# NeLy-EPFL/flygym

Hardware: AMD Instinct MI355X
Metric: env-steps/sec (whole node), 4096 flies per GPU, flat terrain (higher is better)
Workload: dtype f32

## Files before the change

### flygym_amd/csrc/nmf_device.h

```cpp
#pragma once
#include <hip/hip_runtime.h>
#include <stdint.h>

#include <type_traits>
#include <utility>

#include "nmf_families.h"

namespace nmf {

constexpr int kMaxCon = 48;
constexpr int kActHistWords = 64;
constexpr float kMinVal = 1e-15f;

enum { GEOM_CAPSULE = 0, GEOM_HULL = 1 };
enum { ACT_POSITION = 0, ACT_ADHESION = 1, ACT_MOTOR = 2 };

__device__ __forceinline__ int opaque(int v) { asm volatile("" : "+v"(v)); return v; }

template <int... I, class F>
__device__ __forceinline__ void static_for_impl(std::integer_sequence<int, I...>, F&& f) {
  (f(std::integral_constant<int, I>{}), ...);
}
template <int N, class F>
// ... 228 lines not shown
  *cs = ((q + 1) & 2) ? -cc : cc;
}

__device__ __forceinline__ void sym6_add_inertia(Sym6& A, const float* I) {
  A.v[sym_idx(0, 0)] += I[4]; A.v[sym_idx(1, 1)] += I[5]; A.v[sym_idx(2, 2)] += I[6];
  A.v[sym_idx(0, 1)] += I[7]; A.v[sym_idx(0, 2)] += I[8]; A.v[sym_idx(1, 2)] += I[9];
  float hx = I[1], hy = I[2], hz = I[3];
  A.v[sym_idx(0, 4)] += -hz; A.v[sym_idx(0, 5)] += hy;
  A.v[sym_idx(1, 3)] += hz;  A.v[sym_idx(1, 5)] += -hx;
  A.v[sym_idx(2, 3)] += -hy; A.v[sym_idx(2, 4)] += hx;
  A.v[sym_idx(3, 3)] += I[0]; A.v[sym_idx(4, 4)] += I[0]; A.v[sym_idx(5, 5)] += I[0];
}

#define NMF_DPP(v, ctrl) __builtin_bit_cast(float, __builtin_amdgcn_update_dpp(0, __builtin_bit_cast(int, (v)), (ctrl), 0xf, 0xf, true))
#define NMF_PIN(v) asm("" : "+v"(v))
__device__ __forceinline__ float grp8_sum(float v) {
  NMF_PIN(v);
  v += NMF_DPP(v, 0xB1);
  v += NMF_DPP(v, 0x4E);
  v += NMF_DPP(v, 0x141);
  NMF_PIN(v);
  return v;
}

#define NMF_DPP_ROWS(v, ctrl, rows) __builtin_bit_cast(float, __builtin_amdgcn_update_dpp(0, __builtin_bit_cast(int, (v)), (ctrl), (rows), 0xf, false))
__device__ __forceinline__ float wave_sum(float v) {
  v += NMF_DPP(v, 0xB1);
  v += NMF_DPP(v, 0x4E);
  v += NMF_DPP(v, 0x141);
  v += NMF_DPP(v, 0x140);
  v += NMF_DPP_ROWS(v, 0x142, 0xa);
  v += NMF_DPP_ROWS(v, 0x143, 0xc);
  return __builtin_bit_cast(float, __builtin_amdgcn_readlane(__builtin_bit_cast(int, v), 63));
}
template <int I>
__device__ __forceinline__ float grp8_bcast(float v) {
  constexpr int pattern = 0x18 | (I << 5);
  return __builtin_bit_cast(float, __builtin_amdgcn_ds_swizzle(__builtin_bit_cast(int, v), pattern));
}
typedef float f32x4 __attribute__((ext_vector_type(4)));
__device__ __forceinline__ float grp8_lo(float v) {
  return __builtin_bit_cast(float, __builtin_amdgcn_update_dpp(__builtin_bit_cast(int, v), __builtin_bit_cast(int, v), 0x114, 0xf, 0xa, false));
}
__device__ __forceinline__ float grp8_hi(float v) {
  return __builtin_bit_cast(float, __builtin_amdgcn_update_dpp(__builtin_bit_cast(int, v), __builtin_bit_cast(int, v), 0x104, 0xf, 0x5, false));
}
// ... 22 lines not shown
__device__ __forceinline__ int wave_reduce_bits(int v, int idn, Op op) {
  v = op(v, NMF_DPP_OLD(idn, v, 0xB1, 0xf));
  v = op(v, NMF_DPP_OLD(idn, v, 0x4E, 0xf));
  v = op(v, NMF_DPP_OLD(idn, v, 0x141, 0xf));
  v = op(v, NMF_DPP_OLD(idn, v, 0x140, 0xf));
  v = op(v, NMF_DPP_OLD(idn, v, 0x142, 0xa));
  v = op(v, NMF_DPP_OLD(idn, v, 0x143, 0xc));
  return __builtin_amdgcn_readlane(v, 63);
}
__device__ __forceinline__ float wave_min(float v) {
  return __builtin_bit_cast(float, wave_reduce_bits(__builtin_bit_cast(int, v), 0x7f800000, [](int a, int b) {
    return __builtin_bit_cast(int, fminf(__builtin_bit_cast(float, a), __builtin_bit_cast(float, b))); }));
}
__device__ __forceinline__ float wave_max(float v) {
  return __builtin_bit_cast(float, wave_reduce_bits(__builtin_bit_cast(int, v), (int)0xff800000, [](int a, int b) {
    return __builtin_bit_cast(int, fmaxf(__builtin_bit_cast(float, a), __builtin_bit_cast(float, b))); }));
}
__device__ __forceinline__ float groups_sum(float v) {
  v += NMF_DPP(v, 0x128);
  { float a = v, b = v; asm volatile("s_nop 1\n\tv_permlane16_swap_b32 %0, %1\n\ts_nop 1" : "+v"(a), "+v"(b)); v = a + b; }
  { float a = v, b = v; asm volatile("s_nop 1\n\tv_permlane32_swap_b32 %0, %1\n\ts_nop 1" : "+v"(a), "+v"(b)); v = a + b; }
  return v;
}
__device__ __forceinline__ int wave_prefix_min_int(int v) {
  constexpr int big = 0x7fffffff;
  auto mn = [](int a, int b) { return a < b ? a : b; };
  v = mn(v, NMF_DPP_OLD(big, v, 0x111, 0xf));
  v = mn(v, NMF_DPP_OLD(big, v, 0x112, 0xf));
  v = mn(v, NMF_DPP_OLD(big, v, 0x114, 0xf));
  v = mn(v, NMF_DPP_OLD(big, v, 0x118, 0xf));
  v = mn(v, NMF_DPP_OLD(big, v, 0x142, 0xa));
  v = mn(v, NMF_DPP_OLD(big, v, 0x143, 0xc));
  return v;
}
__device__ __forceinline__ int wave_min_int(int v) {
  return wave_reduce_bits(v, 0x7fffffff, [](int a, int b) { return a < b ? a : b; });
}
__device__ __forceinline__ void wave_argmin(float& v, int& i) {
  const float m = wave_min(v);
  i = wave_min_int(v == m ? i : 0x7fffffff);
  v = m;
}
__device__ __forceinline__ void wave_argmax(float& v, int& i) {
  const float m = wave_max(v);
  i = wave_min_int(v == m ? i : 0x7fffffff);
  v = m;
// ... 4 lines not shown
```

### flygym_amd/csrc/nmf_step.hip

```cpp
#include "nmf_device.h"
#include "nmf_step_lds.h"
#include "nmf_step_diag.h"
#include "nmf_tree_fwd.h"
#include "nmf_step_kinematics.h"
#include "nmf_step_collision.h"
#include "nmf_step_aba.h"
#include "nmf_step_contact.h"
#include "nmf_dual.h"
#include "nmf_step_noslip.h"
#include "nmf_step_actuation.h"
#include "nmf_step_forward.h"
#include "nmf_step_io.h"
#include "nmf_tree.h"

namespace nmf {

template <class TP> constexpr int waves_per_simd() { return 2; }

template <class TP>
__device__ __forceinline__ void stage_launch_constants(FlyLds<TP>& s, const GModel& m) {
  if constexpr (!TP::kStar) { if (threadIdx.x == 0) { s.rt_nb = m.nb; s.rt_nv = m.nv; } __syncthreads(); }
  if constexpr (TP::kNFact > 1) {
    for (int b = threadIdx.x; b < TP::kTblB && b < m.nb; b += kWave) {
      s.t_body[b] = (unsigned char)m.tree_body[b < m.tree_lvl_start[m.tree_nlevel] ? b : 0];
      s.t_parent[b] = (unsigned char)(b ? m.body_parent[b] : 0);
      s.t_dofadr[b] = (unsigned char)m.body_dofadr[b]; s.t_dofnum[b] = (unsigned char)m.body_dofnum[b];
      s.t_cstart[b] = (unsigned char)m.tree_child_start[b]; s.t_ccount[b] = (unsigned char)m.tree_child_count[b];
    }
    for (int j = threadIdx.x; j < TP::kTblV && j < m.nv; j += kWave) s.t_dofbody[j] = (unsigned char)m.dof_body[j];
    if (threadIdx.x < 18) s.t_lvl[threadIdx.x] = (unsigned char)m.tree_lvl_start[threadIdx.x];
    if (threadIdx.x == 0) s.t_nlevel = (unsigned char)m.tree_nlevel;
    if constexpr (TP::kStar) {
      for (int i = threadIdx.x; i < kRestLevels * 16; i += kWave) (&s.t_pack[0][0][0])[i] = m.rest_fast ? m.rest_pack[i] : 0xffffffffu;
    }
    __syncthreads();
  }
  const int lane = threadIdx.x;
  for (int j = lane; j < s.nv(); j += kWave) {
    if constexpr (row_width_s<TP>() > 6) s.S[j][6] = 0.f;
    s.arm[j] = m.dof_armature[j];
    if constexpr (kHasCm3<TP>) { s.damp[j] = m.dof_damping[j]; s.dlt[j] = m.dof_armature[j] + m.timestep * m.dof_damping[j]; }
  }
  if (lane < 6) {
    const KLane K = k_lane(lane, make_frame(v3(m.plane[0], m.plane[1], m.plane[2])));
    float* q = s.k_tab[lane];
#pragma unroll
    for (int i = 0; i < 3; ++i) { q[i] = K.dA[i]; q[3 + i] = K.dB[i]; q[6 + i] = K.dO[i]; }
    q[9] = __int_as_float(K.ia); q[10] = __int_as_float(K.ib);
    int words[3];
    inertia_map_pack(lane, words);
    q[11] = __int_as_float(words[0]); q[12] = __int_as_float(words[1]); q[13] = __int_as_float(words[2]);
    if constexpr (kHasIsym<TP>) {
#pragma unroll
      for (int c = 0; c < 6; c++) {
        const int i = lane < c ? lane : c, jx = lane < c ? c : lane;
        q[14 + c] = __int_as_float(sym_idx(i, jx));
      }
    }
  }
  if constexpr (kHasIsym<TP>) if (lane == 0) {
    const Frame fr = make_frame(v3(m.plane[0], m.plane[1], m.plane[2]));
    st3(&s.frame9[0], fr.n); st3(&s.frame9[3], fr.t1); st3(&s.frame9[6], fr.t2);
    HotModel& h = s.hot;
    h.dof_axis = m.dof_axis; h.body_pos = m.body_pos; h.body_quat = m.body_quat; h.geom_p0 = m.geom_p0; h.geom_p1 = m.geom_p1;
// ... 194 lines not shown
```

### flygym_amd/csrc/nmf_step_aba.h

```cpp
#pragma once
#include "nmf_device.h"

namespace nmf {

template <class TP>
__device__ __forceinline__ bool rest_reduced(const FlyLds<TP>& s) {
  if constexpr (TP::kStar) { if constexpr (TP::REST_B > 0) return __builtin_amdgcn_readfirstlane(s.reduced) != 0; }
  return false;
}
template <class TP, class F>
__device__ __forceinline__ void for_dofs(const FlyLds<TP>& s, bool red, int lane, F&& f) {
  if constexpr (TP::kStar) { if constexpr (TP::REST_V > 0) {
    if (red) { for (int jj = lane; jj < TP::NV - TP::REST_V; jj += kWave) f(jj < 6 ? jj : jj + TP::REST_V); return; }
  } }
  for (int j = lane; j < s.nv(); j += kWave) f(j);
}
template <class TP, class F>
__device__ __forceinline__ void for_bodies(const FlyLds<TP>& s, bool red, int lane, F&& f) {
  if constexpr (TP::kStar) { if constexpr (TP::REST_B > 0) {
    if (red) { for (int bb = lane; bb < TP::NB - TP::REST_B; bb += kWave) f(bb < 1 ? 0 : bb + TP::REST_B); return; }
  } }
  for (int b = lane; b < s.nb(); b += kWave) f(b);
}

// ... 45 lines not shown
    float pw[TP::NBL];
#pragma unroll
    for (int l = 0; l < TP::NBL; ++l) pw[l] = W[b0 + l][L.rr];
    static_for<TP::NBL>([&](auto I) {
      constexpr int l = TP::NBL - 1 - decltype(I)::value;
      acc += pw[l];
      W[b0 + l][L.rr] = acc;
    });
  }
  WSYNC();
  if (lane < 6) {
    float a0 = W[0][lane];
#pragma unroll
    for (int k = 0; k < TP::NLEG; ++k) a0 += W[TP::LB0 + k * TP::NBL][lane];
    if constexpr (TP::REST_B > 0) {
      if (!red) for (int k = (int)s.t_cstart[0]; k < (int)s.t_cstart[0] + (int)s.t_ccount[0]; ++k) a0 += W[(int)s.t_body[k]][lane];
    }
    W[0][lane] = a0;
  }
  WSYNC();
  if constexpr (TP::REST_V == 0 && TP::NV > kWave && TP::NV <= 2 * kWave) {
    const int jb = lane + kWave;
    const bool two = jb < TP::NV;
    const float pa = dot(ldsv(s.S[lane]), ldsv(W[dof_body_of<TP>(lane)]));
    float pb = 0.f;
    if (two) pb = dot(ldsv(s.S[jb]), ldsv(W[dof_body_of<TP>(jb)]));
    emit(lane, pa);
    if (two) emit(jb, pb);
  } else {
    for_dofs(s, red, lane, [&](int j) {
      emit(j, dot(ldsv(s.S[j]), ldsv(W[j >= TP::LD0 || j < 6 ? dof_body_of<TP>(j) : tbl_dofbody(s, j)])));
    });
  }
  WSYNC();
  }
}

template <class TP, class Emit>
__device__ __forceinline__ void mul_M(FlyLds<TP>& s, const float* x, const GModel& m, int lane, bool have_twists, Emit&& emit) {
  if (!have_twists) sweep_twists(s, x, s.T, m, lane);
  const bool red = rest_reduced(s);
  for_bodies(s, red, lane, [&](int b) {
    const SV tb = ldsv(s.T[b]);
    SV wb = inert_mul(s.Ib[b], tb);
    if constexpr (TP::kStar) { if constexpr (TP::REST_B > 0) { if (red && b == 0) wb = wb + rest_inertia_mul(s, tb); } }
    stsv(s.W[b], wb);
  });
  WSYNC();
  sweep_project(s, s.W, m, lane, [&](int j, float v) { emit(j, v + s.arm[j] * x[j]); });
}

constexpr int kInertiaIdx[6][6] = {{4, 7, 8, 0, 3, 2}, {7, 5, 9, 3, 0, 1}, {8, 9, 6, 2, 1, 0},
                                   {0, 3, 2, 0, 0, 0}, {3, 0, 1, 0, 0, 0}, {2, 1, 0, 0, 0, 0}};
constexpr int kInertiaSgn[6][6] = {{1, 1, 1, 0, -1, 1}, {1, 1, 1, 1, 0, -1}, {1, 1, 1, -1, 1, 0},
// ... 63 lines not shown
  if constexpr (kHasCm3<TP>) {
    const float* q = s.c_m3[c];
    m_nn = q[0]; m_n1 = q[1]; m_n2 = q[2]; m_11 = q[3]; m_22 = q[4];
    if (m_nn == 0.f) return;
  } else {
    const int act = info_act(s.c_info[c]);
    if (!act) return;
    const float D = s.c_D[c], mu = s.c_mu[c];
    const float a0 = (act & 1) ? 1.f : 0.f, a1 = (act & 2) ? 1.f : 0.f, a2 = (act & 4) ? 1.f : 0.f, a3 = (act & 8) ? 1.f : 0.f;
    const float Dm = D * mu, Dmm = Dm * mu;
    m_nn = D * (a0 + a1 + a2 + a3); m_n1 = Dm * (a0 - a1); m_n2 = Dm * (a2 - a3); m_11 = Dmm * (a0 + a1); m_22 = Dmm * (a2 + a3);
  }
  const V3 rc = ld3(s.c_r[c]);
  const float rcA = s.c_r[c][K.ia], rcB = s.c_r[c][K.ib];
  const float o_n = fmaf(rcA, K.dA[0], fmaf(-rcB, K.dB[0], K.dO[0]));
  const float o_1 = fmaf(rcA, K.dA[1], fmaf(-rcB, K.dB[1], K.dO[1]));
  const float o_2 = fmaf(rcA, K.dA[2], fmaf(-rcB, K.dB[2], K.dO[2]));
  const float C_n = m_nn * o_n + m_n1 * o_1 + m_n2 * o_2, C_1 = m_n1 * o_n + m_11 * o_1, C_2 = m_n2 * o_n + m_22 * o_2;
  const V3 w = C_n * fr.n + C_1 * fr.t1 + C_2 * fr.t2;
  const V3 x = cross(rc, w);
  row[0] += x.x; row[1] += x.y; row[2] += x.z; row[3] += w.x; row[4] += w.y; row[5] += w.z;
}

template <bool MFMA, bool MASKED>
__device__ __forceinline__ void aba_step_core(float (&IA)[6], float& pA, const float* sj, float sown, float mask, float delta, float tauj,
                                              float& U, float& u, float& invD, float& k) {
  f2 a01 = mk2(IA[0], IA[1]), a23 = mk2(IA[2], IA[3]), a45 = mk2(IA[4], IA[5]);
  f2 acc = a01 * mk2(sj[0], sj[1]);
  acc = __builtin_elementwise_fma(a23, mk2(sj[2], sj[3]), acc);
  acc = __builtin_elementwise_fma(a45, mk2(sj[4], sj[5]), acc);
  U = acc.x + acc.y;
  const float sr = MASKED ? mask * sown : sown;
  const float D = grp8_sum(sr * U) + delta;
  const float sp = grp8_sum(sr * pA);
  invD = __builtin_amdgcn_rcpf(D);
  u = tauj - sp;
  k = U * invD;
  if constexpr (MFMA) grp8_rank1_mfma(IA, -k, U);
  else {
    const f2 nk = mk2(-k, -k);
    a01 = __builtin_elementwise_fma(nk, mk2(grp8_bcast<0>(U), grp8_bcast<1>(U)), a01);
    a23 = __builtin_elementwise_fma(nk, mk2(grp8_bcast<2>(U), grp8_bcast<3>(U)), a23);
    a45 = __builtin_elementwise_fma(nk, mk2(grp8_bcast<4>(U), grp8_bcast<5>(U)), a45);
    IA[0] = a01.x; IA[1] = a01.y; IA[2] = a23.x; IA[3] = a23.y; IA[4] = a45.x; IA[5] = a45.y;
  }
  pA += k * u;
}
__device__ __forceinline__ void aba_step(float (&IA)[6], float& pA, const float* sj, float sown, float mask, float delta,
                                         float tauj, float& Uout, float& uout, float& invDout) {
  float U, k;
  aba_step_core<false, true>(IA, pA, sj, sown, mask, delta, tauj, U, uout, invDout, k);
  Uout = mask * U;
}
template <bool SHADOW0, bool MFMA = false>
__device__ __forceinline__ void aba_step_scaled(float (&IA)[6], float& pA, const float* sj, float sr, float mask, float delta,
                                                float tauj, float& UDout, float& uDout, float& Uraw, float& invDraw) {
  float u, k;
  aba_step_core<MFMA, false>(IA, pA, sj, sr, mask, delta, tauj, Uraw, u, invDraw, k);
  UDout = SHADOW0 ? k : mask * k; uDout = u * invDraw;
}
typedef const __attribute__((address_space(3))) float* lds_cptr;
template <class T>
__device__ __forceinline__ lds_cptr lds_pinned(const T* p) {
  lds_cptr q = (lds_cptr)(const void*)p;
  asm("" : "+v"(q));
  return q;
}

template <class TP> __device__ __forceinline__ float (*dual_leg(FlyLds<TP>& s))[8] {
// ... 210 lines not shown
  static_for<TP::NDL>([&](auto DD) {
    constexpr int d = TP::NDL - 1 - decltype(DD)::value;
    float sj[6], row[6];
#pragma unroll
    for (int i = 0; i < 6; i++) { sj[i] = n_sj[i]; row[i] = n_row[i]; }
    const float sown = n_sown, delta = n_delta, delta_e = n_delta_e, tj = n_tau;
    if constexpr (d > 0) fetch_hinge(std::integral_constant<int, (d > 0 ? d - 1 : 0)>{});
    if constexpr (TP::is_last(d)) {
      const int b = b0 + TP::lbody(d);
      if constexpr (kHasIsym<TP>) {
        if constexpr (kDual<TP>) { if (withF) sub_contact_wrenches<true>(pA, s, cs[TP::lbody(d)], cs[TP::lbody(d) + 1], L.rr); }
        if (withK) for (int c = cs[TP::lbody(d)]; c < cs[TP::lbody(d) + 1]; ++c) add_contact_K_row(row, s, c, KL, fr, L.rr, walls);
        add6(IA, row);
        if constexpr (kFuse) add6(IAe, row);
      } else {
        add_inertia_row(IA, s, b, IM);
        if constexpr (kDual<TP>) { if (withF) sub_contact_wrenches<true>(pA, s, cs[TP::lbody(d)], cs[TP::lbody(d) + 1], L.rr); }
        if (withK) for (int c = cs[TP::lbody(d)]; c < cs[TP::lbody(d) + 1]; ++c) add_contact_K_row(IA, s, c, KL, fr, L.rr, walls);
      }
    }
    const float sr = kShadow0 ? sown : L.mask * sown;
    if constexpr (kKeepS) Sreg[d] = sown;
    float Uraw, invDraw;
    aba_step_scaled<kShadow0, kR1>(IA, pA, sj, sr, L.mask, delta, tj, Ureg[d], ureg[d], Uraw, invDraw);
    if constexpr (kFuse) {
      float pe = 0.f, UDe, uDe, Ue, invDe;
      aba_step_scaled<kShadow0, kR1>(IAe, pe, sj, sr, L.mask, delta_e, 0.f, UDe, uDe, Ue, invDe);
      fac[(TP::NDL - 1 - d) * TP::NLEG * 8] = L.r < 6 ? Ue * invDe : invDe;
    }
    if constexpr (kDual<TP>) {
      if (store) {
        const float rs = __builtin_sqrtf(invDraw);
        if constexpr (kDualGlob<TP>) ((__attribute__((address_space(1))) float*)s.dual_glob[0])[(L.lg * TP::NDL + d) * 8 + (L.r < 6 ? L.r : 6)] = L.r < 6 ? Uraw * rs : rs;
        else dual_leg(s)[L.lg * TP::NDL + d][L.r < 6 ? L.r : 6] = L.r < 6 ? Uraw * rs : rs;
      }
    }
  });
  constexpr bool kLegSumValu = TP::NLEG <= 8;
  float legs_row[6] = {0.f, 0.f, 0.f, 0.f, 0.f, 0.f}, legs_pA = 0.f;
  float legs_row_e[6] = {0.f, 0.f, 0.f, 0.f, 0.f, 0.f};
  static_assert(!kFuse || kLegSumValu, "the fused factor sweep sums the legs on the VALU");
  if constexpr (kLegSumValu) {
    const float gm = L.grp < TP::NLEG ? 1.f : 0.f;
#pragma unroll
    for (int i = 0; i < 6; i++) legs_row[i] = groups_sum(gm * IA[i]);
    if constexpr (kFuse) {
#pragma unroll
      for (int i = 0; i < 6; i++) legs_row_e[i] = groups_sum(gm * IAe[i]);
    }
    legs_pA = groups_sum(gm * pA);
  } else {
#pragma unroll
    for (int i = 0; i < 6; i++) H.legIA[L.lg][L.rr][i] = IA[i];
    H.legpA[L.lg][L.rr] = pA;
    WSYNC();
  }
  float Ur[6], ur[6];
  FreeJointAxes R;
  {
    float row[6] = {0.f, 0.f, 0.f, 0.f, 0.f, 0.f};
    if constexpr (kHasIsym<TP>) {
#pragma unroll
      for (int c = 0; c < 6; c++) row[c] = s.Isym[0][so[c]];
    } else add_inertia_row(row, s, 0, IM);
    if (withK) {
      for (int c = cs_root0; c < cs_root1; ++c) add_contact_K_row(row, s, c, KL, fr, L.rr, walls);
      if constexpr (WELD) static_for<6>([&](auto I) { constexpr int i = decltype(I)::value; row[i] += L.rr == i ? s.weldD[i] : 0.f; });
    }
    pA = 0.f;
    if constexpr (kDual<TP>) { if (withF) sub_contact_wrenches<false>(pA, s, cs_root0, cs_root1, L.rr); }
    if constexpr (kFuse) {
#pragma unroll
      for (int i = 0; i < 6; i++) IAe[i] = row[i];
// ... 133 lines not shown
```

### flygym_amd/csrc/nmf_step_contact.h

```cpp
#pragma once
#include "nmf_device.h"

namespace nmf {

template <class TP> constexpr bool dual_hybrid_free() { if constexpr (TP::kStar) return TP::REST_V == 0; else return false; }
template <class TP> constexpr int spring_regs() { if constexpr (dual_hybrid_free<TP>()) return (TP::NV + kWave - 1) / kWave; else return 1; }
struct ContactRegs {
  bool on;
  V3 r;
  int body, geom, info;
  float dist, mu, D, K, B, imp, margin;
  float aref[4], jar[4], jv[4];
};

__device__ __forceinline__ float impedance(const float* si, float r) {
  float d0 = si[0], dmax = si[1], width = si[2], mid = si[3], power = si[4];
  if (d0 == dmax || width <= kMinVal) return 0.5f * (d0 + dmax);
  float x = fabsf(r) / width, y;
  if (x >= 1.f) y = 1.f;
  else if (x <= 0.f) y = 0.f;
  else if (power == 1.f) y = x;
  else if (power == 2.f) y = x <= mid ? x * x / mid : 1.f - (1.f - x) * (1.f - x) / (1.f - mid);
  else if (x <= mid) y = powf(x, power) / powf(mid, power - 1.f);
  else y = 1.f - powf(1.f - x, power) / powf(1.f - mid, power - 1.f);
// ... 84 lines not shown
  float acc = 0.f;
  int cs[TP::NBL + 1];
  static_for<TP::NBL + 1>([&](auto I) { constexpr int l = decltype(I)::value; cs[l] = s.body_cstart[b0 + l]; });
  static_for<TP::NBL>([&](auto I) {
    constexpr int l = TP::NBL - 1 - decltype(I)::value;
    if (SEEDED) acc += seed_scale * s.W[b0 + l][L.rr];
    for (int cc = cs[l]; cc < cs[l + 1]; ++cc) acc += s.c_w[cc][L.rr];
    s.W[b0 + l][L.rr] = acc;
  });
  WSYNC();
  if (lane < 6) {
    float a0 = s.weld_w[lane];
    if (SEEDED) a0 += seed_scale * s.W[0][lane];
    for (int cc = s.body_cstart[0]; cc < s.body_cstart[1]; ++cc) a0 += s.c_w[cc][lane];
#pragma unroll
    for (int k = 0; k < TP::NLEG; ++k) a0 += s.W[TP::LB0 + k * TP::NBL][lane];
    if constexpr (TP::REST_B > 0) {
      if (!red) for (int k = (int)s.t_cstart[0]; k < (int)s.t_cstart[0] + (int)s.t_ccount[0]; ++k) a0 += s.W[(int)s.t_body[k]][lane];
    }
    s.W[0][lane] = a0;
  }
  WSYNC();
  for_dofs(s, red, lane, [&](int j) {
    emit(j, dot(ldsv(s.S[j]), ldsv(s.W[j >= TP::LD0 || j < 6 ? dof_body_of<TP>(j) : tbl_dofbody(s, j)])));
  });
  WSYNC();
  }
}

__device__ __forceinline__ void contact_row_forces(const ContactRegs& c, float sign, float* f) {
#pragma unroll
  for (int k = 0; k < 4; k++) f[k] = c.jar[k] < 0.f ? -sign * c.D * c.jar[k] : 0.f;
}

}
```

### flygym_amd/csrc/nmf_step_kinematics.h

```cpp
#pragma once
#include "nmf_device.h"

namespace nmf {

struct BodyInertial { float q[6], ipos[3], mass; };
__device__ __forceinline__ BodyInertial ld_inertial(const GModel& m, int b) {
  BodyInertial k;
#pragma unroll
  for (int i = 0; i < 6; ++i) k.q[i] = m.body_inertia[6 * b + i];
#pragma unroll
  for (int i = 0; i < 3; ++i) k.ipos[i] = m.body_ipos[3 * b + i];
  k.mass = m.body_mass[b];
  return k;
}
template <class TP>
__device__ __forceinline__ void inertia_of_body(FlyLds<TP>& s, int b, const float* q, const float* ipos, const float* mass) {
  {
    const float* R = s.xmat()[b];
    float Il[9] = {q[0], q[3], q[4], q[3], q[1], q[5], q[4], q[5], q[2]};
    float Tm[9], Iw[9];
#pragma unroll
    for (int i = 0; i < 3; i++)
#pragma unroll
      for (int j = 0; j < 3; j++) Tm[3 * i + j] = R[3 * i] * Il[j] + R[3 * i + 1] * Il[3 + j] + R[3 * i + 2] * Il[6 + j];
#pragma unroll
    for (int i = 0; i < 3; i++)
#pragma unroll
      for (int j = 0; j < 3; j++) Iw[3 * i + j] = Tm[3 * i] * R[3 * j] + Tm[3 * i + 1] * R[3 * j + 1] + Tm[3 * i + 2] * R[3 * j + 2];
    V3 c = mat_vec(R, ld3(ipos)) + (ld3(s.xpos()[b]) - ld3(s.xpos()[0]));
    float ms = *mass, cc = dot(c, c);
    float* I = s.Ib[b];
    I[0] = ms; I[1] = ms * c.x; I[2] = ms * c.y; I[3] = ms * c.z;
    I[4] = Iw[0] + ms * (cc - c.x * c.x); I[5] = Iw[4] + ms * (cc - c.y * c.y); I[6] = Iw[8] + ms * (cc - c.z * c.z);
    I[7] = Iw[1] - ms * c.x * c.y; I[8] = Iw[2] - ms * c.x * c.z; I[9] = Iw[5] - ms * c.y * c.z;
    if constexpr (kHasIsym<TP>) {
      float* Q = s.Isym[b];
      Q[0] = I[4]; Q[1] = I[7]; Q[2] = I[8]; Q[3] = 0.f;   Q[4] = -I[3]; Q[5] = I[2];
      Q[6] = I[5]; Q[7] = I[9]; Q[8] = I[3]; Q[9] = 0.f;   Q[10] = -I[1];
      Q[11] = I[6]; Q[12] = -I[2]; Q[13] = I[1]; Q[14] = 0.f;
      Q[15] = ms; Q[16] = 0.f; Q[17] = 0.f; Q[18] = ms; Q[19] = 0.f; Q[20] = ms;
    }
  }
}

template <class TP>
__device__ __noinline__ void stage_kinematics(FlyLds<TP>& s, const GModel& m, int lane) {
  constexpr int kJq = 5;
  constexpr int kRel = row_width_tw<TP>() > 6 ? 13 : 12;
  float(*jq)[kJq] = reinterpret_cast<float(*)[kJq]>(&s.qacc_smooth[0]);
  float(*relm)[kRel] = reinterpret_cast<float(*)[kRel]>(&s.T[0][0]) - 1;
  float(*axb)[3] = reinterpret_cast<float(*)[3]>(&s.Ib[0][0]);
  static_assert((TP::NB - 1) * kRel <= TP::NB * 2 * row_width_tw<TP>() && TP::NV * 3 <= TP::NB * 10 && kJq <= 6, "kinematics scratch does not fit");
  const HotModel hmk = hot_model(s, m);
  const gptr<float> g_axis = G(hmk.dof_axis), g_quat = G(hmk.body_quat), g_pos = G(hmk.body_pos);
  auto axis_of = [&](int j) { if constexpr (kHasIsym<TP>) return ld3(s.axis[j]); else return ld3(g_axis + 3 * j); };
  BodyInertial inertial;
  if constexpr (kInertiaInKin<TP>) {
    static_assert(!kInertiaInKin<TP> || TP::NB <= kWave, "one body per lane");
    if (lane < s.nb()) inertial = ld_inertial(m, lane);
  }
  for (int j = 6 + lane; j < s.nv(); j += kWave) {
    float sn, cs;
    sincos_bounded(0.5f * s.qpos[j + 1], &sn, &cs);
    const V3 ax = axis_of(j);
    jq[j][0] = cs; jq[j][1] = ax.x * sn; jq[j][2] = ax.y * sn; jq[j][3] = ax.z * sn;
  }
  if (lane == 0) {
    Q4 q = qnorm(ldq(&s.qpos[3]));
    st3(s.xpos()[0], ld3(&s.qpos[0]));
    qmat(s.xmat()[0], q);
  }
  WSYNC();
  for (int b = 1 + lane; b < s.nb(); b += kWave) {
    int adr, num;
    if constexpr (TP::kStar) {
      if (b >= TP::LB0) {
        const int lb = (b - TP::LB0) % TP::NBL;
        adr = TP::LD0 + ((b - TP::LB0) / TP::NBL) * TP::NDL; num = 0;
        static_for<TP::NBL>([&](auto I) { constexpr int l = decltype(I)::value; if (lb == l) { adr += TP::first_dof(l); num = TP::dofs(l); } });
      } else { adr = tbl_dofadr(s, b); num = tbl_dofnum(s, b); }
    } else { adr = tbl_dofadr(s, b); num = tbl_dofnum(s, b); }
    const Q4 bq = ldq(g_quat + 4 * b);
    const V3 bp = ld3(g_pos + 3 * b);
    Q4 P = Q4{1.f, 0.f, 0.f, 0.f};
    for (int j = adr + num - 1; j >= adr; --j) {
      st3(axb[j], qrot_conj(P, axis_of(j)));
      P = qmul(ldq(jq[j]), P);
    }
    qmat(relm[b], qnorm(qmul(bq, P)));
    st3(&relm[b][9], bp);
  }
  WSYNC();
  if constexpr (!TP::kStar) tree_kinematics_chain(s, m, lane, relm);
  else {
    if constexpr (TP::REST_B > 0) tree_kinematics_chain(s, m, lane, relm);
    const LaneRole L = lane_role<TP>(lane);
    const int r3 = L.r < 3 ? L.r : 2;
    float R0 = s.xmat()[0][3 * r3], R1 = s.xmat()[0][3 * r3 + 1], R2 = s.xmat()[0][3 * r3 + 2];
    float p = s.xpos()[0][r3];
// ... 2 lines not shown
#pragma unroll
    for (int k = 0; k < 12; ++k) Mn[k] = relm[b0][k];
    static_for<TP::NBL>([&](auto I) {
      constexpr int l = decltype(I)::value;
      float M[12];
#pragma unroll
      for (int k = 0; k < 12; ++k) M[k] = Mn[k];
      p += R0 * M[9] + R1 * M[10] + R2 * M[11];
      const float n0 = R0 * M[0] + R1 * M[3] + R2 * M[6];
      const float n1 = R0 * M[1] + R1 * M[4] + R2 * M[7];
      const float n2 = R0 * M[2] + R1 * M[5] + R2 * M[8];
      R0 = n0; R1 = n1; R2 = n2;
      if constexpr (l + 1 < TP::NBL) {
#pragma unroll
        for (int k = 0; k < 12; ++k) Mn[k] = relm[b0 + l + 1][k];
        __builtin_amdgcn_sched_barrier(0);
      }
      s.xmat()[b0 + l][3 * r3] = R0; s.xmat()[b0 + l][3 * r3 + 1] = R1; s.xmat()[b0 + l][3 * r3 + 2] = R2;
      s.xpos()[b0 + l][r3] = p;
    });
  }
  WSYNC();
  for (int j = lane; j < s.nv(); j += kWave) {
    SV S;
    if (j < 3) {
      S.a = v3(0.f, 0.f, 0.f);
      S.l = v3(j == 0 ? 1.f : 0.f, j == 1 ? 1.f : 0.f, j == 2 ? 1.f : 0.f);
    } else if (j < 6) {
      int c = j - 3;
      S.a = v3(s.xmat()[0][c], s.xmat()[0][3 + c], s.xmat()[0][6 + c]);
      S.l = v3(0.f, 0.f, 0.f);
    } else {
      int b;
      if constexpr (TP::kStar) b = j >= TP::LD0 ? dof_body_of<TP>(j) : tbl_dofbody(s, j); else b = tbl_dofbody(s, j);
      V3 a = mat_vec(s.xmat()[b], ld3(axb[j]));
      V3 r = ld3(s.xpos()[0]) - ld3(s.xpos()[b]);
      S.a = a;
      S.l = cross(a, r);
    }
    stsv(s.S[j], S);
  }
  WSYNC();
  if constexpr (kInertiaInKin<TP>) {
    if (lane < s.nb()) inertia_of_body(s, lane, inertial.q, inertial.ipos, &inertial.mass);
    WSYNC();
  }
}

template <class TP>
__device__ void stage_inertia(FlyLds<TP>& s, const GModel& m, int lane) {
  for (int b = lane; b < s.nb(); b += kWave) {
    const float* R = s.xmat()[b];
    const float* q = &m.body_inertia[6 * b];
    float Il[9] = {q[0], q[3], q[4], q[3], q[1], q[5], q[4], q[5], q[2]};
    float Tm[9], Iw[9];
#pragma unroll
    for (int i = 0; i < 3; i++)
#pragma unroll
      for (int j = 0; j < 3; j++) Tm[3 * i + j] = R[3 * i] * Il[j] + R[3 * i + 1] * Il[3 + j] + R[3 * i + 2] * Il[6 + j];
#pragma unroll
    for (int i = 0; i < 3; i++)
#pragma unroll
      for (int j = 0; j < 3; j++) Iw[3 * i + j] = Tm[3 * i] * R[3 * j] + Tm[3 * i + 1] * R[3 * j + 1] + Tm[3 * i + 2] * R[3 * j + 2];
    V3 c = mat_vec(R, ld3(&m.body_ipos[3 * b])) + (ld3(s.xpos()[b]) - ld3(s.xpos()[0]));
    float ms = m.body_mass[b], cc = dot(c, c);
    float* I = s.Ib[b];
    I[0] = ms; I[1] = ms * c.x; I[2] = ms * c.y; I[3] = ms * c.z;
    I[4] = Iw[0] + ms * (cc - c.x * c.x); I[5] = Iw[4] + ms * (cc - c.y * c.y); I[6] = Iw[8] + ms * (cc - c.z * c.z);
    I[7] = Iw[1] - ms * c.x * c.y; I[8] = Iw[2] - ms * c.x * c.z; I[9] = Iw[5] - ms * c.y * c.z;
    if constexpr (kHasIsym<TP>) {
      float* Q = s.Isym[b];
      Q[0] = I[4]; Q[1] = I[7]; Q[2] = I[8]; Q[3] = 0.f;   Q[4] = -I[3]; Q[5] = I[2];
      Q[6] = I[5]; Q[7] = I[9]; Q[8] = I[3]; Q[9] = 0.f;   Q[10] = -I[1];
      Q[11] = I[6]; Q[12] = -I[2]; Q[13] = I[1]; Q[14] = 0.f;
      Q[15] = ms; Q[16] = 0.f; Q[17] = 0.f; Q[18] = ms; Q[19] = 0.f; Q[20] = ms;
    }
  }
  WSYNC();
}

}
```

### flygym_amd/csrc/nmf_step_lds.h

```cpp
#pragma once
#include "nmf_device.h"

namespace nmf {

#define WSYNC() do { __builtin_amdgcn_fence(__ATOMIC_SEQ_CST, "wavefront"); __builtin_amdgcn_wave_barrier(); } while (0)
constexpr float kNoiseFactor = 8.f;
enum : unsigned int {
  kExitDual = 1u << 8,
  kExitKkt = 1u << 9,
  kExitTie = 1u << 10,
  kExitStall = 1u << 11,
  kExitCost = 1u << 12,
  kExitMaxIter = 1u << 13,
  kExitPrimal = 1u << 14,
  kExitFallback = 1u << 15,
  kExitBigPivots = 1u << 16,
  kExitNoNoslip = 1u << 17,
  kExitFree = 1u << 18,
};
constexpr int kExitKinds = 12;
constexpr int kDualRegPivots = 47;
constexpr float kDualResidMax = 1e-3f;
constexpr int kDualExitFrom = 5;

// ... 62 lines not shown
#ifdef NMF_STEP_FIXED_OLD
  return false;
#else
  if constexpr (TP::kStar) return !(TP::REST_B > 0 && TP::kTerrain); else return true;
#endif
}
template <class TP> constexpr bool inertia_in_kinematics() {
#ifdef NMF_STEP_FIXED_OLD
  return false;
#else
  return has_cm3<TP>() && !TP::kTerrain;
#endif
}
template <class TP> inline constexpr bool kStepCursor = step_cursor<TP>();
template <class TP> inline constexpr bool kInertiaInKin = inertia_in_kinematics<TP>();
template <class TP> constexpr bool aba_rank1_mfma() {
#ifdef NMF_ABA_RANK1_VALU
  return false;
#else
  return euler_fused<TP>();
#endif
}
template <class TP> inline constexpr bool kAbaRank1Mfma = aba_rank1_mfma<TP>();
template <class TP> constexpr int euler_scratch_floats() { if constexpr (has_cm3<TP>()) return 8 * (TP::NLEG * TP::NDL + 6); else return 0; }
constexpr int dual_g_floats(int ncon) { return 9 * ncon * (ncon + 1) / 2; }
template <class TP> constexpr int dual_max_con() {
  if constexpr (kDualH<TP>) {
    int n = 0;
    while (n < 16 && dual_g_floats(n + 1) <= 2 * TP::NB * 6) ++n;
    return n;
  } else return 16;
}
template <class TP> inline constexpr int kDualMaxCon = dual_max_con<TP>();
template <class TP> inline constexpr int kHistLds = kDualS<TP> ? kActHistWords : kDualH<TP> ? 5 : 0;
template <class TP, class M> __device__ __forceinline__ int hist_words(const M& m) {
  if constexpr (kDualS<TP>) return (m.ng + 1) / 2; else return kHistLds<TP>;
}
template <class TP> constexpr int dual_pad_floats() {
  if constexpr (kDualS<TP>) {
    constexpr int need = dual_g_floats(kDualMaxCon<TP>);
    constexpr int have = TP::NB * 11 + 2 * TP::NB * (TP::REST_B == 0 ? conflict_free_width(TP::NBL, TP::NLEG) : 6);
    return need > have ? need - have : 0;
  } else return 0;
}

struct HotModel {
// ... 37 lines not shown
  float c_r[kMaxCon][3], c_D[kMaxCon], c_mu[kMaxCon];
  int c_info[kMaxCon];
  alignas(kDualS<TP> ? 16 : 4) float xpos_pad_[kDualS<TP> ? 1 : 0];
  float xpos_root[3];
  float c_w[kMaxCon][7];
  float c_m3[kHasCm3<TP> ? kMaxCon : 1][kHasCm3<TP> ? 5 : 1];
  float k_tab[6][kHasIsym<TP> ? 20 : 14];
  float frame9[kHasIsym<TP> ? 9 : 1];
  std::conditional_t<kHasIsym<TP>, HotModel, char> hot;
  float axis[kHasIsym<TP> ? TP::NV : 1][3];
  float weldD[6], weld_w[6];
  using cstart_t = std::conditional_t<kHasIsym<TP>, int, unsigned char>;
  cstart_t body_cstart[(TP::NB + 1 + 3) / 4 * 4];
  __device__ __forceinline__ float* slot_at(int k) {
    if constexpr (TP::kStar) {
      constexpr int kInCw = 7 * kMaxCon / 27;
      static_assert(TP::REST_B == 0 || (TP::REST_B - kInCw) * 27 * sizeof(float) + sizeof(AbaHandoff<TP>) <= sizeof(float) * TP::NB * 2 * row_width_tw<TP>(),
                    "hand-off slots of the rest do not fit T..W");
      return k < kInCw ? &c_w[0][0] + 27 * k : &T[0][0] + sizeof(AbaHandoff<TP>) / sizeof(float) + 27 * (k - kInCw);
    } else return this->slot[k];
  }
  unsigned int act_hist[kHistLds<TP>];
  float* dual_glob[kDualGlob<TP> ? 1 : 0];
  int ncon, overflow;
  int iters;
  float solve_resid;
  int nwall;
  __device__ __forceinline__ float* vec(int id) {
    switch (id) {
      case 0: return qacc;
      case 1: return qacc_smooth;
      case 2: return qfrc_smooth;
      case 3: return vA;
      case 4: return vB;
      case 5: return vC;
      default: return vD;
    }
  }
};
template <class TP> __device__ __forceinline__ HotModel hot_model(const FlyLds<TP>& s, const GModel& m) {
  if constexpr (kHasIsym<TP>) return s.hot;
  else {
    HotModel h;
    h.dof_axis = (const float*)m.dof_axis; h.body_pos = (const float*)m.body_pos; h.body_quat = (const float*)m.body_quat;
    h.geom_p0 = (const float*)m.geom_p0; h.geom_p1 = (const float*)m.geom_p1; h.geom_radius = (const float*)m.geom_radius;
    h.geom_bsphere = (const float*)m.geom_bsphere; h.hull_vert = (const float*)m.hull_vert; h.pair_margin = (const float*)m.pair_margin;
// ... 50 lines not shown
  if constexpr (sizeof(s.frame9) == 9 * sizeof(float)) return Frame{ld3(&s.frame9[0]), ld3(&s.frame9[3]), ld3(&s.frame9[6])};
  else return make_frame(v3(m.plane[0], m.plane[1], m.plane[2]));
}

__device__ __forceinline__ Frame contact_frame(int fid, const Frame& f0) {
  const float sg = (fid & 1) ? 1.f : -1.f;
  const bool xw = fid <= 2, pl = fid == 0;
  Frame f;
  f.n = pl ? f0.n : (xw ? v3(sg, 0.f, 0.f) : v3(0.f, sg, 0.f));
  f.t1 = pl ? f0.t1 : (xw ? v3(0.f, 1.f, 0.f) : v3(0.f, 0.f, 1.f));
  f.t2 = pl ? f0.t2 : (xw ? v3(0.f, 0.f, sg) : v3(sg, 0.f, 0.f));
  return f;
}

template <class TP>
__device__ __forceinline__ int dof_body_of(int j) {
  if (j < 6) return 0;
  const int leg = (j - TP::LD0) / TP::NDL, d = (j - TP::LD0) % TP::NDL;
  int lb = 0;
  static_for<TP::NBL - 1>([&](auto I) { constexpr int l = decltype(I)::value; lb += d >= TP::first_dof(l + 1) ? 1 : 0; });
  return TP::LB0 + leg * TP::NBL + lb;
}

struct LaneRole {
  int grp, r, lg, rr;
  bool live;
  float mask;
};
template <class TP>
__device__ __forceinline__ LaneRole lane_role(int lane) {
  LaneRole L;
  L.grp = lane >> 3; L.r = lane & 7;
  L.lg = L.grp < TP::NLEG ? L.grp : TP::NLEG - 1;
  L.rr = L.r < 6 ? L.r : 5;
  L.live = L.grp < TP::NLEG && L.r < 6;
  L.mask = L.r < 6 ? 1.f : 0.f;
  return L;
}

}
```

Baseline: 65.84 million.

## Batch lane reductions, fuse paired ABA steps, add LDS index tables and launch constants

Interleaves several independent DPP and permlane reductions (grp8_sum2/3, groups_sum_n) so their latencies overlap instead of serialising. Fuses the main and shadow ABA factor steps into one paired step that shares a single three-way group reduction. Replaces the per-call integer div/mod computation of dof-to-body and body-dof ranges with byte lookup tables in LDS. Moves the constant entries of Isym and the first three motion subspace rows to launch time so they are not rewritten every step. The cost is more LDS use and more live registers, which could lower occupancy.

```diff
diff --git a/flygym_amd/csrc/nmf_device.h b/flygym_amd/csrc/nmf_device.h
--- a/flygym_amd/csrc/nmf_device.h
+++ b/flygym_amd/csrc/nmf_device.h
@@ -274,6 +274,28 @@
   NMF_PIN(v);
   return v;
 }
+__device__ __forceinline__ void grp8_sum2(float& a, float& b) {
+#ifdef NMF_ISSUE_OLD
+  a = grp8_sum(a); b = grp8_sum(b);
+#else
+  NMF_PIN(a); NMF_PIN(b);
+  a += NMF_DPP(a, 0xB1);  b += NMF_DPP(b, 0xB1);
+  a += NMF_DPP(a, 0x4E);  b += NMF_DPP(b, 0x4E);
+  a += NMF_DPP(a, 0x141); b += NMF_DPP(b, 0x141);
+  NMF_PIN(a); NMF_PIN(b);
+#endif
+}
+__device__ __forceinline__ void grp8_sum3(float& a, float& b, float& c) {
+#ifdef NMF_ISSUE_OLD
+  a = grp8_sum(a); b = grp8_sum(b); c = grp8_sum(c);
+#else
+  NMF_PIN(a); NMF_PIN(b); NMF_PIN(c);
+  a += NMF_DPP(a, 0xB1);  b += NMF_DPP(b, 0xB1);  c += NMF_DPP(c, 0xB1);
+  a += NMF_DPP(a, 0x4E);  b += NMF_DPP(b, 0x4E);  c += NMF_DPP(c, 0x4E);
+  a += NMF_DPP(a, 0x141); b += NMF_DPP(b, 0x141); c += NMF_DPP(c, 0x141);
+  NMF_PIN(a); NMF_PIN(b); NMF_PIN(c);
+#endif
+}
 
 #define NMF_DPP_ROWS(v, ctrl, rows) __builtin_bit_cast(float, __builtin_amdgcn_update_dpp(0, __builtin_bit_cast(int, (v)), (ctrl), (rows), 0xf, false))
 __device__ __forceinline__ float wave_sum(float v) {
@@ -342,6 +364,48 @@
   { float a = v, b = v; asm volatile("s_nop 1\n\tv_permlane32_swap_b32 %0, %1\n\ts_nop 1" : "+v"(a), "+v"(b)); v = a + b; }
   return v;
 }
+#define NMF_SWAP_1(op, i) "\n\t" op " %[a" #i "], %[b" #i "]"
+#define NMF_SWAP_2(op, i, j) NMF_SWAP_1(op, i) NMF_SWAP_1(op, j)
+#define NMF_SWAP_V(i) [a##i] "+v"(a[i]), [b##i] "+v"(b[i])
+template <int K, bool HALVES>
+__device__ __forceinline__ void groups_swap_add(float* a) {
+  float b[K];
+#pragma unroll
+  for (int i = 0; i < K; i++) b[i] = a[i];
+#define NMF_SWAP_BLOCK(body, ...) \
+  if constexpr (HALVES) asm volatile("s_nop 1" body("v_permlane32_swap_b32") "\n\ts_nop 1" : __VA_ARGS__); \
+  else asm volatile("s_nop 1" body("v_permlane16_swap_b32") "\n\ts_nop 1" : __VA_ARGS__)
+#define NMF_SWAP_B1(op) NMF_SWAP_1(op, 0)
+#define NMF_SWAP_B2(op) NMF_SWAP_2(op, 0, 1)
+#define NMF_SWAP_B4(op) NMF_SWAP_B2(op) NMF_SWAP_2(op, 2, 3)
+#define NMF_SWAP_B8(op) NMF_SWAP_B4(op) NMF_SWAP_2(op, 4, 5) NMF_SWAP_2(op, 6, 7)
+  static_assert(K == 1 || K == 2 || K == 4 || K == 8, "block sizes");
+  if constexpr (K == 1) { NMF_SWAP_BLOCK(NMF_SWAP_B1, NMF_SWAP_V(0)); }
+  else if constexpr (K == 2) { NMF_SWAP_BLOCK(NMF_SWAP_B2, NMF_SWAP_V(0), NMF_SWAP_V(1)); }
+  else if constexpr (K == 4) { NMF_SWAP_BLOCK(NMF_SWAP_B4, NMF_SWAP_V(0), NMF_SWAP_V(1), NMF_SWAP_V(2), NMF_SWAP_V(3)); }
+  else { NMF_SWAP_BLOCK(NMF_SWAP_B8, NMF_SWAP_V(0), NMF_SWAP_V(1), NMF_SWAP_V(2), NMF_SWAP_V(3), NMF_SWAP_V(4), NMF_SWAP_V(5), NMF_SWAP_V(6), NMF_SWAP_V(7)); }
+#undef NMF_SWAP_BLOCK
+#pragma unroll
+  for (int i = 0; i < K; i++) a[i] = a[i] + b[i];
+}
+template <int N, bool HALVES>
+__device__ __forceinline__ void groups_swap_stage(float* v) {
+  constexpr int K = N >= 8 ? 8 : N >= 4 ? 4 : N >= 2 ? 2 : 1;
+  groups_swap_add<K, HALVES>(v);
+  if constexpr (N > K) groups_swap_stage<N - K, HALVES>(v + K);
+}
+template <int N>
+__device__ __forceinline__ void groups_sum_n(float (&v)[N]) {
+#ifdef NMF_ISSUE_OLD
+#pragma unroll
+  for (int i = 0; i < N; i++) v[i] = groups_sum(v[i]);
+#else
+#pragma unroll
+  for (int i = 0; i < N; i++) v[i] += NMF_DPP(v[i], 0x128);
+  groups_swap_stage<N, false>(v);
+  groups_swap_stage<N, true>(v);
+#endif
+}
 __device__ __forceinline__ int wave_prefix_min_int(int v) {
   constexpr int big = 0x7fffffff;
   auto mn = [](int a, int b) { return a < b ? a : b; };
diff --git a/flygym_amd/csrc/nmf_step.hip b/flygym_amd/csrc/nmf_step.hip
--- a/flygym_amd/csrc/nmf_step.hip
+++ b/flygym_amd/csrc/nmf_step.hip
@@ -40,6 +40,29 @@
     if constexpr (row_width_s<TP>() > 6) s.S[j][6] = 0.f;
     s.arm[j] = m.dof_armature[j];
     if constexpr (kHasCm3<TP>) { s.damp[j] = m.dof_damping[j]; s.dlt[j] = m.dof_armature[j] + m.timestep * m.dof_damping[j]; }
+  }
+  if constexpr (kLaneTables<TP>) {
+    static_assert(!kLaneTables<TP> || (TP::LD0 == 6 && TP::LB0 == 1 && TP::NB <= 256 && TP::NV <= 256), "byte tables of a leg-chain skeleton");
+    for (int j = lane; j < TP::NV; j += kWave) s.dof_body_tab[j] = (unsigned char)dof_body_of<TP>(j);
+    for (int b = lane; b < TP::NB; b += kWave) {
+      int adr = 0, num = 0;
+      if (b >= TP::LB0) leg_body_dofs<TP>(b, adr, num);
+      s.body_adr_tab[b] = (unsigned char)adr; s.body_num_tab[b] = (unsigned char)num;
+    }
+  }
+  if constexpr (kLaunchWords<TP>) {
+    if (lane < 3) {
+      SV S;
+      S.a = v3(0.f, 0.f, 0.f);
+      S.l = v3(lane == 0 ? 1.f : 0.f, lane == 1 ? 1.f : 0.f, lane == 2 ? 1.f : 0.f);
+      stsv(s.S[lane], S);
+    }
+    for (int b = lane; b < TP::NB; b += kWave) {
+      float* Q = s.Isym[b];
+      const float ms = m.body_mass[b];
+      Q[3] = 0.f; Q[9] = 0.f; Q[14] = 0.f;
+      Q[15] = ms; Q[16] = 0.f; Q[17] = 0.f; Q[18] = ms; Q[19] = 0.f; Q[20] = ms;
+    }
   }
   if (lane < 6) {
     const KLane K = k_lane(lane, make_frame(v3(m.plane[0], m.plane[1], m.plane[2])));
diff --git a/flygym_amd/csrc/nmf_step_aba.h b/flygym_amd/csrc/nmf_step_aba.h
--- a/flygym_amd/csrc/nmf_step_aba.h
+++ b/flygym_amd/csrc/nmf_step_aba.h
@@ -91,14 +91,14 @@
   if constexpr (TP::REST_V == 0 && TP::NV > kWave && TP::NV <= 2 * kWave) {
     const int jb = lane + kWave;
     const bool two = jb < TP::NV;
-    const float pa = dot(ldsv(s.S[lane]), ldsv(W[dof_body_of<TP>(lane)]));
+    const float pa = dot(ldsv(s.S[lane]), ldsv(W[dof_body_at(s, lane)]));
     float pb = 0.f;
-    if (two) pb = dot(ldsv(s.S[jb]), ldsv(W[dof_body_of<TP>(jb)]));
+    if (two) pb = dot(ldsv(s.S[jb]), ldsv(W[dof_body_at(s, jb)]));
     emit(lane, pa);
     if (two) emit(jb, pb);
   } else {
     for_dofs(s, red, lane, [&](int j) {
-      emit(j, dot(ldsv(s.S[j]), ldsv(W[j >= TP::LD0 || j < 6 ? dof_body_of<TP>(j) : tbl_dofbody(s, j)])));
+      emit(j, dot(ldsv(s.S[j]), ldsv(W[j >= TP::LD0 || j < 6 ? dof_body_at(s, j) : tbl_dofbody(s, j)])));
     });
   }
   WSYNC();
@@ -208,9 +208,29 @@
   row[0] += x.x; row[1] += x.y; row[2] += x.z; row[3] += w.x; row[4] += w.y; row[5] += w.z;
 }
 
+__device__ __forceinline__ float aba_row_product(const float (&IA)[6], const float* sj) {
+  const f2 a01 = mk2(IA[0], IA[1]), a23 = mk2(IA[2], IA[3]), a45 = mk2(IA[4], IA[5]);
+  f2 acc = a01 * mk2(sj[0], sj[1]);
+  acc = __builtin_elementwise_fma(a23, mk2(sj[2], sj[3]), acc);
+  acc = __builtin_elementwise_fma(a45, mk2(sj[4], sj[5]), acc);
+  return acc.x + acc.y;
+}
+template <bool MFMA>
+__device__ __forceinline__ void aba_downdate(float (&IA)[6], float U, float k) {
+  if constexpr (MFMA) grp8_rank1_mfma(IA, -k, U);
+  else {
+    f2 a01 = mk2(IA[0], IA[1]), a23 = mk2(IA[2], IA[3]), a45 = mk2(IA[4], IA[5]);
+    const f2 nk = mk2(-k, -k);
+    a01 = __builtin_elementwise_fma(nk, mk2(grp8_bcast<0>(U), grp8_bcast<1>(U)), a01);
+    a23 = __builtin_elementwise_fma(nk, mk2(grp8_bcast<2>(U), grp8_bcast<3>(U)), a23);
+    a45 = __builtin_elementwise_fma(nk, mk2(grp8_bcast<4>(U), grp8_bcast<5>(U)), a45);
+    IA[0] = a01.x; IA[1] = a01.y; IA[2] = a23.x; IA[3] = a23.y; IA[4] = a45.x; IA[5] = a45.y;
+  }
+}
 template <bool MFMA, bool MASKED>
 __device__ __forceinline__ void aba_step_core(float (&IA)[6], float& pA, const float* sj, float sown, float mask, float delta, float tauj,
                                               float& U, float& u, float& invD, float& k) {
+#ifdef NMF_ISSUE_OLD
   f2 a01 = mk2(IA[0], IA[1]), a23 = mk2(IA[2], IA[3]), a45 = mk2(IA[4], IA[5]);
   f2 acc = a01 * mk2(sj[0], sj[1]);
   acc = __builtin_elementwise_fma(a23, mk2(sj[2], sj[3]), acc);
@@ -231,6 +251,34 @@
     IA[0] = a01.x; IA[1] = a01.y; IA[2] = a23.x; IA[3] = a23.y; IA[4] = a45.x; IA[5] = a45.y;
   }
   pA += k * u;
+#else
+  U = aba_row_product(IA, sj);
+  const float sr = MASKED ? mask * sown : sown;
+  float Dsum = sr * U, sp = sr * pA;
+  grp8_sum2(Dsum, sp);
+  const float D = Dsum + delta;
+  invD = __builtin_amdgcn_rcpf(D);
+  u = tauj - sp;
+  k = U * invD;
+  aba_downdate<MFMA>(IA, U, k);
+  pA += k * u;
+#endif
+}
+template <bool MFMA>
+__device__ __forceinline__ void aba_step_pair(float (&IA)[6], float& pA, float (&IAe)[6], const float* sj, float sr, float delta, float delta_e,
+                                              float tauj, float& U, float& u, float& invD, float& k, float& Ue, float& invDe) {
+  U = aba_row_product(IA, sj);
+  Ue = aba_row_product(IAe, sj);
+  float Dsum = sr * U, sp = sr * pA, De = sr * Ue;
+  grp8_sum3(Dsum, sp, De);
+  const float D = Dsum + delta;
+  invD = __builtin_amdgcn_rcpf(D);
+  u = tauj - sp;
+  k = U * invD;
+  aba_downdate<MFMA>(IA, U, k);
+  pA += k * u;
+  invDe = __builtin_amdgcn_rcpf(De + delta_e);
+  aba_downdate<MFMA>(IAe, Ue, Ue * invDe);
 }
 __device__ __forceinline__ void aba_step(float (&IA)[6], float& pA, const float* sj, float sown, float mask, float delta,
                                          float tauj, float& Uout, float& uout, float& invDout) {
@@ -487,11 +535,23 @@
     const float sr = kShadow0 ? sown : L.mask * sown;
     if constexpr (kKeepS) Sreg[d] = sown;
     float Uraw, invDraw;
+#ifdef NMF_ISSUE_OLD
+    constexpr bool kPair = false;
+#else
+    constexpr bool kPair = kFuse;
+#endif
+    if constexpr (kPair) {
+      float u, k, Ue, invDe;
+      aba_step_pair<kR1>(IA, pA, IAe, sj, sr, delta, delta_e, tj, Uraw, u, invDraw, k, Ue, invDe);
+      Ureg[d] = kShadow0 ? k : L.mask * k; ureg[d] = u * invDraw;
+      fac[(TP::NDL - 1 - d) * TP::NLEG * 8] = L.r < 6 ? Ue * invDe : invDe;
+    } else {
     aba_step_scaled<kShadow0, kR1>(IA, pA, sj, sr, L.mask, delta, tj, Ureg[d], ureg[d], Uraw, invDraw);
     if constexpr (kFuse) {
       float pe = 0.f, UDe, uDe, Ue, invDe;
       aba_step_scaled<kShadow0, kR1>(IAe, pe, sj, sr, L.mask, delta_e, 0.f, UDe, uDe, Ue, invDe);
       fac[(TP::NDL - 1 - d) * TP::NLEG * 8] = L.r < 6 ? Ue * invDe : invDe;
+    }
     }
     if constexpr (kDual<TP>) {
       if (store) {
@@ -507,6 +567,7 @@
   static_assert(!kFuse || kLegSumValu, "the fused factor sweep sums the legs on the VALU");
   if constexpr (kLegSumValu) {
     const float gm = L.grp < TP::NLEG ? 1.f : 0.f;
+#ifdef NMF_ISSUE_OLD
 #pragma unroll
     for (int i = 0; i < 6; i++) legs_row[i] = groups_sum(gm * IA[i]);
     if constexpr (kFuse) {
@@ -514,6 +575,24 @@
       for (int i = 0; i < 6; i++) legs_row_e[i] = groups_sum(gm * IAe[i]);
     }
     legs_pA = groups_sum(gm * pA);
+#else
+    float leg_sums[kFuse ? 13 : 7];
+#pragma unroll
+    for (int i = 0; i < 6; i++) leg_sums[i] = gm * IA[i];
+    leg_sums[6] = gm * pA;
+    if constexpr (kFuse) {
+#pragma unroll
+      for (int i = 0; i < 6; i++) leg_sums[7 + i] = gm * IAe[i];
+    }
+    groups_sum_n(leg_sums);
+#pragma unroll
+    for (int i = 0; i < 6; i++) legs_row[i] = leg_sums[i];
+    legs_pA = leg_sums[6];
+    if constexpr (kFuse) {
+#pragma unroll
+      for (int i = 0; i < 6; i++) legs_row_e[i] = leg_sums[7 + i];
+    }
+#endif
   } else {
 #pragma unroll
     for (int i = 0; i < 6; i++) H.legIA[L.lg][L.rr][i] = IA[i];
diff --git a/flygym_amd/csrc/nmf_step_contact.h b/flygym_amd/csrc/nmf_step_contact.h
--- a/flygym_amd/csrc/nmf_step_contact.h
+++ b/flygym_amd/csrc/nmf_step_contact.h
@@ -130,7 +130,7 @@
   }
   WSYNC();
   for_dofs(s, red, lane, [&](int j) {
-    emit(j, dot(ldsv(s.S[j]), ldsv(s.W[j >= TP::LD0 || j < 6 ? dof_body_of<TP>(j) : tbl_dofbody(s, j)])));
+    emit(j, dot(ldsv(s.S[j]), ldsv(s.W[j >= TP::LD0 || j < 6 ? dof_body_at(s, j) : tbl_dofbody(s, j)])));
   });
   WSYNC();
   }
diff --git a/flygym_amd/csrc/nmf_step_kinematics.h b/flygym_amd/csrc/nmf_step_kinematics.h
--- a/flygym_amd/csrc/nmf_step_kinematics.h
+++ b/flygym_amd/csrc/nmf_step_kinematics.h
@@ -35,10 +35,16 @@
     I[7] = Iw[1] - ms * c.x * c.y; I[8] = Iw[2] - ms * c.x * c.z; I[9] = Iw[5] - ms * c.y * c.z;
     if constexpr (kHasIsym<TP>) {
       float* Q = s.Isym[b];
+      if constexpr (kLaunchWords<TP>) {
+        Q[0] = I[4]; Q[1] = I[7]; Q[2] = I[8]; Q[4] = -I[3]; Q[5] = I[2];
+        Q[6] = I[5]; Q[7] = I[9]; Q[8] = I[3]; Q[10] = -I[1];
+        Q[11] = I[6]; Q[12] = -I[2]; Q[13] = I[1];
+      } else {
       Q[0] = I[4]; Q[1] = I[7]; Q[2] = I[8]; Q[3] = 0.f;   Q[4] = -I[3]; Q[5] = I[2];
       Q[6] = I[5]; Q[7] = I[9]; Q[8] = I[3]; Q[9] = 0.f;   Q[10] = -I[1];
       Q[11] = I[6]; Q[12] = -I[2]; Q[13] = I[1]; Q[14] = 0.f;
       Q[15] = ms; Q[16] = 0.f; Q[17] = 0.f; Q[18] = ms; Q[19] = 0.f; Q[20] = ms;
+      }
     }
   }
 }
@@ -74,7 +80,8 @@
   for (int b = 1 + lane; b < s.nb(); b += kWave) {
     int adr, num;
     if constexpr (TP::kStar) {
-      if (b >= TP::LB0) {
+      if constexpr (kLaneTables<TP>) { adr = s.body_adr_tab[b]; num = s.body_num_tab[b]; }
+      else if (b >= TP::LB0) {
         const int lb = (b - TP::LB0) % TP::NBL;
         adr = TP::LD0 + ((b - TP::LB0) / TP::NBL) * TP::NDL; num = 0;
         static_for<TP::NBL>([&](auto I) { constexpr int l = decltype(I)::value; if (lb == l) { adr += TP::first_dof(l); num = TP::dofs(l); } });
@@ -123,6 +130,7 @@
   }
   WSYNC();
   for (int j = lane; j < s.nv(); j += kWave) {
+    if constexpr (kLaunchWords<TP>) { if (j < 3) continue; }
     SV S;
     if (j < 3) {
       S.a = v3(0.f, 0.f, 0.f);
@@ -133,7 +141,7 @@
       S.l = v3(0.f, 0.f, 0.f);
     } else {
       int b;
-      if constexpr (TP::kStar) b = j >= TP::LD0 ? dof_body_of<TP>(j) : tbl_dofbody(s, j); else b = tbl_dofbody(s, j);
+      if constexpr (TP::kStar) b = j >= TP::LD0 ? dof_body_at(s, j) : tbl_dofbody(s, j); else b = tbl_dofbody(s, j);
       V3 a = mat_vec(s.xmat()[b], ld3(axb[j]));
       V3 r = ld3(s.xpos()[0]) - ld3(s.xpos()[b]);
       S.a = a;
@@ -171,10 +179,16 @@
     I[7] = Iw[1] - ms * c.x * c.y; I[8] = Iw[2] - ms * c.x * c.z; I[9] = Iw[5] - ms * c.y * c.z;
     if constexpr (kHasIsym<TP>) {
       float* Q = s.Isym[b];
+      if constexpr (kLaunchWords<TP>) {
+        Q[0] = I[4]; Q[1] = I[7]; Q[2] = I[8]; Q[4] = -I[3]; Q[5] = I[2];
+        Q[6] = I[5]; Q[7] = I[9]; Q[8] = I[3]; Q[10] = -I[1];
+        Q[11] = I[6]; Q[12] = -I[2]; Q[13] = I[1];
+      } else {
       Q[0] = I[4]; Q[1] = I[7]; Q[2] = I[8]; Q[3] = 0.f;   Q[4] = -I[3]; Q[5] = I[2];
       Q[6] = I[5]; Q[7] = I[9]; Q[8] = I[3]; Q[9] = 0.f;   Q[10] = -I[1];
       Q[11] = I[6]; Q[12] = -I[2]; Q[13] = I[1]; Q[14] = 0.f;
       Q[15] = ms; Q[16] = 0.f; Q[17] = 0.f; Q[18] = ms; Q[19] = 0.f; Q[20] = ms;
+      }
     }
   }
   WSYNC();
diff --git a/flygym_amd/csrc/nmf_step_lds.h b/flygym_amd/csrc/nmf_step_lds.h
--- a/flygym_amd/csrc/nmf_step_lds.h
+++ b/flygym_amd/csrc/nmf_step_lds.h
@@ -108,6 +108,15 @@
 #endif
 }
 template <class TP> inline constexpr bool kAbaRank1Mfma = aba_rank1_mfma<TP>();
+template <class TP> constexpr bool lane_tables() {
+#ifdef NMF_ISSUE_OLD
+  return false;
+#else
+  return has_cm3<TP>();
+#endif
+}
+template <class TP> inline constexpr bool kLaneTables = lane_tables<TP>();
+template <class TP> inline constexpr bool kLaunchWords = lane_tables<TP>();
 template <class TP> constexpr int euler_scratch_floats() { if constexpr (has_cm3<TP>()) return 8 * (TP::NLEG * TP::NDL + 6); else return 0; }
 constexpr int dual_g_floats(int ncon) { return 9 * ncon * (ncon + 1) / 2; }
 template <class TP> constexpr int dual_max_con() {
@@ -191,6 +200,7 @@
   }
   unsigned int act_hist[kHistLds<TP>];
   float* dual_glob[kDualGlob<TP> ? 1 : 0];
+  unsigned char dof_body_tab[kLaneTables<TP> ? TP::NV : 0], body_adr_tab[kLaneTables<TP> ? TP::NB : 0], body_num_tab[kLaneTables<TP> ? TP::NB : 0];
   int ncon, overflow;
   int iters;
   float solve_resid;
@@ -287,6 +297,17 @@
   return TP::LB0 + leg * TP::NBL + lb;
 }
 
+template <class TP>
+__device__ __forceinline__ void leg_body_dofs(int b, int& adr, int& num) {
+  const int lb = (b - TP::LB0) % TP::NBL;
+  adr = TP::LD0 + ((b - TP::LB0) / TP::NBL) * TP::NDL; num = 0;
+  static_for<TP::NBL>([&](auto I) { constexpr int l = decltype(I)::value; if (lb == l) { adr += TP::first_dof(l); num = TP::dofs(l); } });
+}
+template <class TP>
+__device__ __forceinline__ int dof_body_at(const FlyLds<TP>& s, int j) {
+  if constexpr (kLaneTables<TP>) return s.dof_body_tab[j]; else return dof_body_of<TP>(j);
+}
+
 struct LaneRole {
   int grp, r, lg, rr;
   bool live;
```

Result: no change. 66.30 million, median of 6 (+0.7%).
